# blyssprivacy/sdk

Measured on NVIDIA H100. Metric: PIR server queries/sec (Spiral process_query), higher is better.
Workload: dtype u64

## Files before the change

### sdk_b200/build.py

```python
import os
import subprocess
import sys

HERE = os.path.dirname(os.path.abspath(__file__))
CSRC = os.path.join(HERE, "csrc")
SO = os.path.join(HERE, "libb200pir.so")
SOURCES = ["api.cu", "poly_kernels.cu", "mul_kernels.cu", "imma_kernels.cu", "wire_kernels.cu", "tc5_kernels.cu", "dpir_gemm.cu"]
HEADERS = ["common.cuh", "kernels.h", "ntt_core.cuh", "tc5_layout.cuh", "tc5_ptx.cuh", "ntt_core4096.cuh", "ntt_tables.hpp",
           "item_place.cuh", "update_body.hpp", os.path.join("..", "..", "include", "b200pir.h")]
NVCC_FLAGS = ["-gencode", "arch=compute_90a,code=sm_90a", "-lineinfo", "-O3", "-std=c++17", "--extended-lambda",
              "-Xcompiler", "-fPIC", "-ccbin", "/usr/bin/g++" if os.path.exists("/usr/bin/g++") else "g++"]


def _stale():
    if not os.path.exists(SO):
        return True
    t = os.path.getmtime(SO)
    return any(os.path.getmtime(os.path.join(CSRC, f)) > t for f in SOURCES + HEADERS)


def build(force=False, verbose=False):
    if not force and not _stale():
        return SO
    nvcc = os.environ.get("NVCC", "/usr/local/cuda/bin/nvcc")
    objs = []
    procs = []
    for src in SOURCES:
        obj = os.path.join(CSRC, src.replace(".cu", ".o"))
        cmd = [nvcc] + NVCC_FLAGS + (["-Xptxas", "-v"] if verbose else []) + ["-c", os.path.join(CSRC, src), "-o", obj]
        procs.append((src, subprocess.Popen(cmd, stdout=subprocess.PIPE, stderr=subprocess.STDOUT, text=True)))
        objs.append(obj)
    for src, p in procs:
        out, _ = p.communicate()
        if verbose or p.returncode:
            sys.stderr.write(out)
        if p.returncode:
            raise RuntimeError("nvcc failed on " + src)
    subprocess.check_call([nvcc, "-shared", "-gencode", "arch=compute_90a,code=sm_90a", "-o", SO] + objs + ["-ccbin", NVCC_FLAGS[-1]])
    return SO


if __name__ == "__main__":
    print(build(force="--force" in sys.argv, verbose="-v" in sys.argv))
```

### sdk_b200/csrc/poly_kernels.cu

```cuda
#include "kernels.h"
#include "ntt_core4096.cuh"

namespace b200pir {

namespace {

constexpr int CTA = 512;
constexpr int HI_TW = NTT_N - 64;

__constant__ Twiddle c_tw_lo[2][3][64];

struct TwConst {
  int n, dir;
  __device__ __forceinline__ Twiddle operator()(int i) const { return c_tw_lo[n][dir][i]; }
  __device__ __forceinline__ void load2(int i, Twiddle (&t)[2]) const { t[0] = (*this)(i); t[1] = (*this)(i + 1); }
  __device__ __forceinline__ void load4(int i, Twiddle (&t)[4]) const {
    t[0] = (*this)(i); t[1] = (*this)(i + 1); t[2] = (*this)(i + 2); t[3] = (*this)(i + 3);
  }
};
struct TwShared {
  const Twiddle* p;
  __device__ __forceinline__ Twiddle operator()(int i) const { return p[i - 64]; }
  __device__ __forceinline__ void load2(int i, Twiddle (&t)[2]) const {
    uint4 v = *reinterpret_cast<const uint4*>(p + (i - 64));
    t[0] = Twiddle{v.x, v.y}; t[1] = Twiddle{v.z, v.w};
  }
  __device__ __forceinline__ void load4(int i, Twiddle (&t)[4]) const {
    uint4 v = *reinterpret_cast<const uint4*>(p + (i - 64)), w = *(reinterpret_cast<const uint4*>(p + (i - 64)) + 1);
    t[0] = Twiddle{v.x, v.y}; t[1] = Twiddle{v.z, v.w}; t[2] = Twiddle{w.x, w.y}; t[3] = Twiddle{w.z, w.w};
  }
};
struct TwGlobal {
  const Twiddle* p;
  __device__ __forceinline__ Twiddle operator()(int i) const {
    uint2 v = __ldg(reinterpret_cast<const uint2*>(p + i));
    return Twiddle{v.x, v.y};
  }
  __device__ __forceinline__ void load2(int i, Twiddle (&t)[2]) const {
    uint4 v = __ldg(reinterpret_cast<const uint4*>(p + i));
    t[0] = Twiddle{v.x, v.y}; t[1] = Twiddle{v.z, v.w};
  }
  __device__ __forceinline__ void load4(int i, Twiddle (&t)[4]) const {
    uint4 v = __ldg(reinterpret_cast<const uint4*>(p + i)), w = __ldg(reinterpret_cast<const uint4*>(p + i) + 1);
    t[0] = Twiddle{v.x, v.y}; t[1] = Twiddle{v.z, v.w}; t[2] = Twiddle{w.x, w.y}; t[3] = Twiddle{w.z, w.w};
  }
};

struct Grp {
  int tid;
  int n;
  uint32_t q;
  uint64_t cr1;
  const Twiddle* fwd;
  const Twiddle* inv;
  const Twiddle* inv_lz;
  uint32_t* smem;
  uint32_t* smem2;
  const Twiddle* fwd_hi_sm;
};
struct CtaSync {
  __device__ __forceinline__ void operator()() const { __syncthreads(); }
};

__device__ __forceinline__ Grp make_grp(const DevParams& P, uint32_t* ntt_smem) {
  Grp g;
  g.n = threadIdx.x >> 8;
  g.tid = threadIdx.x & 255;
  g.q = g.n ? P.q[1] : P.q[0];
  g.cr1 = g.n ? P.cr1[1] : P.cr1[0];
  g.fwd = g.n ? P.fwd[1] : P.fwd[0];
  g.inv = g.n ? P.inv[1] : P.inv[0];
  g.inv_lz = g.n ? P.inv_lz[1] : P.inv_lz[0];
  g.smem = ntt_smem + g.n * NTT_SMEM_WORDS;
  g.smem2 = nullptr;
  g.fwd_hi_sm = nullptr;
  return g;
}
__device__ __forceinline__ Grp make_grp_single(const DevParams& P, uint32_t* ntt_smem, int n) {
  Grp g;
  g.n = n;
  g.tid = threadIdx.x;
  g.q = n ? P.q[1] : P.q[0];
  g.cr1 = n ? P.cr1[1] : P.cr1[0];
  g.fwd = n ? P.fwd[1] : P.fwd[0];
  g.inv = n ? P.inv[1] : P.inv[0];
  g.inv_lz = n ? P.inv_lz[1] : P.inv_lz[0];
  g.smem = ntt_smem;
  g.smem2 = nullptr;
  g.fwd_hi_sm = nullptr;
  return g;
}
__device__ __forceinline__ void stage_fwd_twiddles(Grp& g, Twiddle* dst) {
  for (int i = g.tid; i < HI_TW; i += 256) {
    uint2 v = __ldg(reinterpret_cast<const uint2*>(g.fwd + 64 + i));
    dst[i] = Twiddle{v.x, v.y};
  }
  g.fwd_hi_sm = dst;
// ... 57 lines not shown
      for (int a = 0; a < 8; a++) {
        const uint64_t va = v(a);
        x0[a] = gadget_digit_fast<BYTE>(va, k, bits, mask);
        x1[a] = gadget_digit_fast<BYTE>(va, k + 1, bits, mask);
      }
      ntt_forward_group2_lz<NTT_OUT_LAZY16>(g.tid, x0, x1, g.smem, g.smem2, TwConst{g.n, 0}, TwShared{g.fwd_hi_sm}, g.q, CtaSync());
      if (cnt + 2 > 16) { acc_reduce<ROWS>(acc, g); cnt = 1; }
      cnt += 2;
      const uint32_t* c = c0 + (size_t)k * col_step;
#pragma unroll
      for (int r = 0; r < ROWS; r++) {
        uint32_t cv[8];
        ld8_ro(cv, c + (size_t)r * row_step);
#pragma unroll
        for (int e = 0; e < 8; e++) acc[r][e] += (uint64_t)x0[e] * cv[e];
      }
#pragma unroll
      for (int r = 0; r < ROWS; r++) {
        uint32_t cv[8];
        ld8_ro(cv, c + col_step + (size_t)r * row_step);
#pragma unroll
        for (int e = 0; e < 8; e++) acc[r][e] += (uint64_t)x1[e] * cv[e];
      }
    }
  }
#pragma unroll 1
  for (; k < ndig; k++) {
    uint32_t x[8];
#pragma unroll
    for (int a = 0; a < 8; a++) x[a] = gadget_digit_fast<BYTE>(v(a), k, bits, mask);
    if (SM) ntt_forward_group_lz<NTT_OUT_LAZY16>(g.tid, x, g.smem, TwConst{g.n, 0}, TwShared{g.fwd_hi_sm}, g.q, CtaSync());
    else ntt_forward_group_lz<NTT_OUT_LAZY16>(g.tid, x, g.smem, TwConst{g.n, 0}, TwGlobal{g.fwd}, g.q, CtaSync());
    if (cnt + 1 > 16) { acc_reduce<ROWS>(acc, g); cnt = 1; }
    cnt += 1;
    const uint32_t* c = c0 + (size_t)k * col_step;
#pragma unroll
    for (int r = 0; r < ROWS; r++) {
      uint32_t cv[8];
      ld8_ro(cv, c + (size_t)r * row_step);
#pragma unroll
      for (int e = 0; e < 8; e++) acc[r][e] += (uint64_t)x[e] * cv[e];
    }
  }
}

template <int ROWS, bool SM, typename Coef>
__device__ __forceinline__ void digits_mac(uint64_t (&acc)[ROWS][8], int& cnt, Coef v, int ndig,
                                           int bits, const uint32_t* c0, size_t col_step, size_t row_step,
                                           const Grp& g) {
  if (bits == 8) digits_mac_impl<ROWS, SM, true>(acc, cnt, v, ndig, bits, c0, col_step, row_step, g);
  else digits_mac_impl<ROWS, SM, false>(acc, cnt, v, ndig, bits, c0, col_step, row_step, g);
}

template <typename Sink>
__device__ __forceinline__ void crt_lift(const uint32_t (&x)[8], uint32_t* res, const Grp& g, const DevParams& P,
                                         Sink sink) {
  __syncthreads();
#pragma unroll
  for (int a = 0; a < 8; a++) res[g.n * POLY + a * 256 + g.tid] = x[a];
  __syncthreads();
#pragma unroll
  for (int a4 = 0; a4 < 4; a4++) {
    int z = (g.n * 4 + a4) * 256 + g.tid;
    sink(z, crt_compose(res[z], res[POLY + z], P));
  }
}

__global__ void __launch_bounds__(256) k_ntt32(DevParams P, uint32_t* polys, int inverse) {
  __shared__ __align__(16) uint32_t ntt_smem[NTT_SMEM_WORDS];
  Grp g = make_grp_single(P, ntt_smem, blockIdx.y);
  uint32_t* p = polys + ((size_t)blockIdx.x * 2 + g.n) * POLY;
  uint32_t x[8];
  if (!inverse) {
#pragma unroll
    for (int a = 0; a < 8; a++) x[a] = p[a * 256 + g.tid];
    grp_ntt_fwd<false>(g, x);
    st8(p + g.tid * 8, x);
  } else {
    ld8(x, p + g.tid * 8);
    grp_ntt_inv(g, x);
#pragma unroll
    for (int a = 0; a < 8; a++) p[a * 256 + g.tid] = x[a];
  }
}
__global__ void __launch_bounds__(NTT4K_THREADS)
k_ntt32_4k(uint32_t q0, uint32_t q1, const Twiddle* __restrict__ tw , uint32_t* polys, int inverse) {
  __shared__ __align__(16) uint32_t sm[NTT4K_SMEM_WORDS];
  const int n = blockIdx.y, tid = threadIdx.x;
  const uint32_t q = n ? q1 : q0;
  uint32_t* p = polys + ((size_t)blockIdx.x * 2 + n) * NTT4K_N;
  const TwGlobal tab{tw + (size_t)(2 * n + (inverse ? 1 : 0)) * NTT4K_N};
  uint32_t x[8];
  if (!inverse) {
#pragma unroll
    for (int a = 0; a < 8; a++) x[a] = p[a * NTT4K_THREADS + tid];
    ntt4k_forward_group(tid, x, sm, tab, q, CtaSync());
    st8(p + tid * 8, x);
  } else {
    ld8(x, p + tid * 8);
    ntt4k_inverse_group(tid, x, sm, tab, q, CtaSync());
#pragma unroll
    for (int a = 0; a < 8; a++) p[a * NTT4K_THREADS + tid] = x[a];
  }
}
__global__ void __launch_bounds__(256) k_ntt_u64(DevParams P, uint64_t* polys, int inverse) {
  __shared__ __align__(16) uint32_t ntt_smem[NTT_SMEM_WORDS];
// ... 67 lines not shown
             size_t c_batch_stride, int slices_per_query, int t_gsw, int bits) {
  __shared__ __align__(16) uint32_t ntt_smem[2 * NTT_SMEM_WORDS];
  __shared__ uint32_t res[2 * POLY];
  Grp g = make_grp(P, ntt_smem);
  const int b = blockIdx.x / half, i = blockIdx.x % half;
  uint64_t* base = cts + (size_t)b * batch_stride;
  const size_t qoff = (size_t)(b / slices_per_query) * c_batch_stride;
  const int cols = 2 * t_gsw;
  const size_t col_step = (size_t)2 * 2 * POLY;
  const size_t row_step = (size_t)cols * 2 * POLY;

  uint64_t acc[2][8];
#pragma unroll
  for (int r = 0; r < 2; r++)
#pragma unroll
    for (int e = 0; e < 8; e++) acc[r][e] = 0;
  int cnt = 0;
#pragma unroll 1
  for (int src = 0; src < 2; src++) {
    const uint64_t* ct = base + (size_t)(src == 0 ? i : half + i) * 2 * POLY;
    const uint32_t* C = (src == 0 ? c_neg : c_pos) + qoff;
#pragma unroll 1
    for (int rho = 0; rho < 2; rho++) {
      uint64_t v[8];
#pragma unroll
      for (int a = 0; a < 8; a++) v[a] = ct[rho * POLY + a * 256 + g.tid];
      const uint32_t* c0 = C + ((size_t)rho * 2 + g.n) * POLY + g.tid * 8;
      digits_mac<2, false>(acc, cnt, RegCoef{v}, t_gsw, bits, c0, col_step, row_step, g);
    }
  }
  uint64_t* dst = base + (size_t)i * 2 * POLY;
#pragma unroll 1
  for (int r = 0; r < 2; r++) {
    uint32_t x[8];
#pragma unroll
    for (int e = 0; e < 8; e++) x[e] = barrett64(acc[r][e], g.cr1, g.q);
    grp_ntt_inv(g, x);
    uint64_t* d = dst + r * POLY;
    crt_lift(x, res, g, P, [&](int z, uint64_t val) { d[z] = val; });
  }
}

__device__ __forceinline__ uint32_t digit_diff(uint64_t vh, uint64_t vi, int k, int bits, uint64_t mask, uint32_t q) {
  return gadget_digit(vh, k, bits, mask) - gadget_digit(vi, k, bits, mask) + q;
}
__device__ __forceinline__ uint32_t byte_pair_diff(uint64_t vh, uint64_t vi, int k) {
  const uint32_t sel = 0x7070u | ((uint32_t)(k + 1) << 8) | (uint32_t)k;
  return __byte_perm((uint32_t)vh, (uint32_t)(vh >> 32), sel) + 0x01000100u -
         __byte_perm((uint32_t)vi, (uint32_t)(vi >> 32), sel);
}
constexpr int kFoldPlanes = 4;

template <bool BYTE>
__global__ void __launch_bounds__(256, 2)
k_fold_res_lz(DevParams P, const uint32_t* __restrict__ in, uint32_t* __restrict__ out, size_t batch_stride, int half,
              const uint32_t* __restrict__ c_pos, size_t c_batch_stride, int slices_per_query, int t_gsw, int bits,
              const uint32_t* __restrict__ zero_flags ) {
  if (zero_flags) {
    const int bz = blockIdx.x / half, iz = blockIdx.x % half;
    const uint32_t fa = zero_flags[(size_t)bz * 2 * half + iz], fb = zero_flags[(size_t)bz * 2 * half + half + iz];
    if (fa | fb) {
      const uint32_t* src = in + (size_t)bz * batch_stride + (size_t)((fa ? half : 0) + iz) * 4 * POLY;
      uint32_t* dst = out + (size_t)bz * batch_stride + (size_t)iz * 4 * POLY;
#pragma unroll
      for (int rho = 0; rho < 2; rho++) {
        uint32_t x[8];
        ld8_ro(x, src + ((size_t)rho * 2 + blockIdx.y) * POLY + threadIdx.x * 8);
        st8(dst + ((size_t)rho * 2 + blockIdx.y) * POLY + threadIdx.x * 8, x);
      }
      return;
    }
  }
  extern __shared__ __align__(16) uint8_t dyn_smem[];
  uint32_t* sm0 = reinterpret_cast<uint32_t*>(dyn_smem);
  uint32_t* sm1 = sm0 + NTT_SMEM_WORDS;
  Twiddle* tw = reinterpret_cast<Twiddle*>(sm1 + NTT_SMEM_WORDS);
  Grp g = make_grp_single(P, sm0, blockIdx.y);
  stage_fwd_twiddles(g, tw);
  const TwConst lo{g.n, 0};
  const TwShared hi{tw};
  const int b = blockIdx.x / half, i = blockIdx.x % half;
  const uint32_t* ci = in + (size_t)b * batch_stride + (size_t)i * 4 * POLY;
  const uint32_t* ch = in + (size_t)b * batch_stride + (size_t)(half + i) * 4 * POLY;
  const uint32_t* C = c_pos + (size_t)(b / slices_per_query) * c_batch_stride;
  const int cols = 2 * t_gsw;
  const size_t row_step = (size_t)cols * 2 * POLY;
  const uint64_t mask = (1ull << bits) - 1;
  const uint32_t q = g.q;
  uint32_t* planes = reinterpret_cast<uint32_t*>(tw + HI_TW) + g.tid;

  uint64_t acc[2][8];
#pragma unroll
  for (int r = 0; r < 2; r++)
#pragma unroll
    for (int e = 0; e < 8; e++) acc[r][e] = 0;
  int cnt = 0;
#pragma unroll 1
  for (int rho = 0; rho < 2; rho++) {
    uint64_t vi[8], vh[8];
#pragma unroll
    for (int a = 0; a < 8; a++) {
      const int z = a * 256 + g.tid;
      vi[a] = crt_compose(__ldg(ci + (rho * 2 + 0) * POLY + z), __ldg(ci + (rho * 2 + 1) * POLY + z), P);
      vh[a] = crt_compose(__ldg(ch + (rho * 2 + 0) * POLY + z), __ldg(ch + (rho * 2 + 1) * POLY + z), P);
      if (BYTE) {
#pragma unroll
        for (int p = 0; p < kFoldPlanes; p++)
          if (2 * p < t_gsw) planes[p * POLY + a * 256] = byte_pair_diff(vh[a], vi[a], 2 * p);
      }
    }
    const uint32_t* c0 = C + ((size_t)rho * 2 + g.n) * POLY + g.tid * 8;
    int k = 0;
#pragma unroll 1
    for (; k + 1 < t_gsw; k += 2) {
      uint32_t x0[8], x1[8];
#pragma unroll
      for (int a = 0; a < 8; a++) {
        if (BYTE) {
          const uint32_t w = planes[(k >> 1) * POLY + a * 256];
          x0[a] = (w & 0xffffu) + (q - 256u);
          x1[a] = (w >> 16) + (q - 256u);
        } else {
          x0[a] = digit_diff(vh[a], vi[a], k, bits, mask, q);
          x1[a] = digit_diff(vh[a], vi[a], k + 1, bits, mask, q);
        }
      }
      ntt_forward_group2_lz<NTT_OUT_LAZY16>(g.tid, x0, x1, sm0, sm1, lo, hi, q, CtaSync());
      if (cnt + 2 > 16) { acc_reduce<2>(acc, g); cnt = 1; }
      cnt += 2;
#pragma unroll
      for (int r = 0; r < 2; r++) {
        uint32_t cv[8];
        ld8_ro(cv, c0 + (size_t)r * row_step + (size_t)k * 4 * POLY);
#pragma unroll
        for (int e = 0; e < 8; e++) acc[r][e] += (uint64_t)x0[e] * cv[e];
      }
#pragma unroll
      for (int r = 0; r < 2; r++) {
        uint32_t cv[8];
        ld8_ro(cv, c0 + (size_t)r * row_step + (size_t)(k + 1) * 4 * POLY);
#pragma unroll
        for (int e = 0; e < 8; e++) acc[r][e] += (uint64_t)x1[e] * cv[e];
      }
    }
    if (k < t_gsw) {
      uint32_t x0[8];
#pragma unroll
      for (int a = 0; a < 8; a++)
        x0[a] = BYTE ? (planes[(k >> 1) * POLY + a * 256] & 0xffffu) + (q - 256u) : digit_diff(vh[a], vi[a], k, bits, mask, q);
      ntt_forward_group_lz<NTT_OUT_LAZY16>(g.tid, x0, sm0, lo, hi, q, CtaSync());
      if (cnt + 1 > 16) { acc_reduce<2>(acc, g); cnt = 1; }
      cnt += 1;
#pragma unroll
      for (int r = 0; r < 2; r++) {
        uint32_t cv[8];
        ld8_ro(cv, c0 + (size_t)r * row_step + (size_t)k * 4 * POLY);
#pragma unroll
        for (int e = 0; e < 8; e++) acc[r][e] += (uint64_t)x0[e] * cv[e];
      }
    }
  }
  uint32_t y0[8], y1[8];
#pragma unroll
  for (int e = 0; e < 8; e++) {
    y0[e] = barrett64(acc[0][e], g.cr1, q);
    y1[e] = barrett64(acc[1][e], g.cr1, q);
  }
  ntt_inverse_group2_nh(g.tid, y0, y1, sm0, sm1, TwConst{g.n, 2}, TwGlobal{g.inv_lz}, q, CtaSync());
  uint32_t* co = out + (size_t)b * batch_stride + (size_t)i * 4 * POLY;
#pragma unroll
  for (int a = 0; a < 8; a++) {
    const int z = a * 256 + g.tid;
    co[(0 * 2 + g.n) * POLY + z] = addmod(y0[a], __ldg(ci + (0 * 2 + g.n) * POLY + z), q);
    co[(1 * 2 + g.n) * POLY + z] = addmod(y1[a], __ldg(ci + (1 * 2 + g.n) * POLY + z), q);
  }
}

__global__ void __launch_bounds__(256)
k_ct_zero_flags(const uint32_t* __restrict__ cts, size_t batch_stride, int per_batch, uint32_t* __restrict__ flags) {
  const int b = blockIdx.x / per_batch, idx = blockIdx.x % per_batch;
  const uint4* p = reinterpret_cast<const uint4*>(cts + (size_t)b * batch_stride + (size_t)idx * 4 * POLY);
  uint32_t acc = 0;
#pragma unroll
  for (int k = 0; k < 8; k++) {
    const uint4 v = __ldg(p + k * 256 + threadIdx.x);
    acc |= v.x | v.y | v.z | v.w;
  }
  const int any = __syncthreads_or(acc != 0);
  if (threadIdx.x == 0) flags[blockIdx.x] = any ? 0u : 1u;
}

__global__ void k_folding_neg(DevParams P, uint32_t* out, const uint32_t* vf, size_t total, int t_gsw, int bits) {
  size_t idx = (size_t)blockIdx.x * blockDim.x + threadIdx.x;
  if (idx >= total) return;
  int n = (int)((idx / POLY) & 1);
  size_t poly = idx / (2 * POLY);
  int cols = 2 * t_gsw;
  int c = (int)(poly % cols);
  int r = (int)((poly / cols) & 1);
  uint32_t q = P.q[n];
  uint32_t v = vf[idx];
  uint32_t neg = v == 0 ? 0u : q - v;
  uint32_t gval = 0;
  if ((c & 1) == r) {
    int j = c >> 1;
    if (bits * j < 64) gval = barrett64(1ull << (bits * j), P.cr1[n], q);
  }
  out[idx] = addmod(neg, gval, q);
}

__global__ void k_expand_scalar(DevParams P, uint32_t* v, size_t v_stride, int num_in, const uint32_t* neg1) {
  v += (size_t)blockIdx.y * v_stride;
  size_t idx = (size_t)blockIdx.x * blockDim.x + threadIdx.x;
  size_t total = (size_t)num_in * 4 * POLY;
  if (idx >= total) return;
  int z = (int)(idx % POLY);
  int n = (int)((idx / POLY) & 1);
  uint32_t a = v[idx], b = neg1[n * POLY + z];
  v[total + idx] = barrett64((uint64_t)a * b, P.cr1[n], P.q[n]);
}

__global__ void __launch_bounds__(CTA, 1) k_expand_round(DevParams P, uint32_t* v, size_t v_stride, ExpandRound R) {
  v += (size_t)blockIdx.y * v_stride;
  extern __shared__ __align__(16) uint8_t dyn_smem[];
  uint32_t* ntt_smem = reinterpret_cast<uint32_t*>(dyn_smem);
  uint32_t* res = ntt_smem + 4 * NTT_SMEM_WORDS;
  uint64_t* autom = reinterpret_cast<uint64_t*>(res + 2 * POLY);
// ... 467 lines not shown

__device__ __forceinline__ uint64_t rescale_dev(uint64_t a, uint64_t inp_mod, uint64_t out_mod) {
  typedef __int128 i128;
  long long inp_mod_i = (long long)inp_mod;
  long long inp_val = (long long)(a % inp_mod);
  if (inp_val >= inp_mod_i / 2) inp_val -= inp_mod_i;
  long long sign = inp_val >= 0 ? 1 : -1;
  i128 val = (i128)inp_val * (i128)out_mod;
  i128 result = (val + (i128)(sign * (inp_mod_i / 2))) / (i128)inp_mod;
  i128 om = (i128)out_mod;
  result = (result + (i128)((inp_mod / out_mod) * out_mod) + 2 * om) % om;
  return (uint64_t)((result + om) % om);
}
__global__ void k_encode(DevParams P, uint64_t* out, size_t out_words, const uint64_t* packed, size_t packed_q_stride, int n,
                         int instances, uint64_t q2, int q2_bits, uint64_t q1, int q1_bits) {
  size_t w = (size_t)blockIdx.x * blockDim.x + threadIdx.x;
  if (w >= out_words) return;
  out += (size_t)blockIdx.y * out_words;
  packed += (size_t)blockIdx.y * packed_q_stride;
  const uint64_t first_cnt = (uint64_t)n * POLY, rest_cnt = (uint64_t)n * n * POLY;
  const uint64_t inst_bits = first_cnt * q2_bits + rest_cnt * q1_bits;
  uint64_t lo_bit = (uint64_t)w * 64, hi_bit = lo_bit + 64;
  uint64_t word = 0;
  uint64_t bit = lo_bit;
  while (bit < hi_bit) {
    uint64_t inst = bit / inst_bits;
    if (inst >= (uint64_t)instances) break;
    uint64_t off = bit - inst * inst_bits;
    const uint64_t* pk = packed + inst * (uint64_t)(n + 1) * n * POLY;
    uint64_t vstart, val;
    int vb;
    if (off < first_cnt * q2_bits) {
      uint64_t vi = off / q2_bits;
      vstart = inst * inst_bits + vi * q2_bits;
      vb = q2_bits;
      val = rescale_dev(pk[vi], P.modulus, q2);
    } else {
      uint64_t o2 = off - first_cnt * q2_bits;
      uint64_t vi = o2 / q1_bits;
      vstart = inst * inst_bits + first_cnt * q2_bits + vi * q1_bits;
      vb = q1_bits;
      val = rescale_dev(pk[first_cnt + vi], P.modulus, q1);
    }
    val &= (vb >= 64) ? ~0ull : ((1ull << vb) - 1);
    if (vstart >= lo_bit) word |= val << (vstart - lo_bit);
    else word |= val >> (lo_bit - vstart);
    bit = vstart + vb;
  }
  out[w] = word;
}

inline unsigned grid1d(size_t total, int block) { return (unsigned)((total + block - 1) / block); }
const size_t kDynSmemBig = (size_t)(4 * NTT_SMEM_WORDS + 2 * POLY) * 4 + (size_t)2 * POLY * 8 + (size_t)2 * HI_TW * 8;
const size_t kDynSmemFold = (size_t)(2 * NTT_SMEM_WORDS) * 4 + (size_t)HI_TW * 8;

}

void upload_poly_constants(const Twiddle* lo ) {
  B200_CUDA(cudaMemcpyToSymbol(c_tw_lo, lo, sizeof(Twiddle) * 2 * 3 * 64));
}
void launch_ntt_u64(const DevParams& P, uint64_t* polys, size_t count, bool inverse, cudaStream_t s) {
  if (count) ++g_kernel_launches, k_ntt_u64<<<dim3((unsigned)count, 2), 256, 0, s>>>(P, polys, inverse ? 1 : 0);
}
void launch_ntt32(const DevParams& P, uint32_t* polys, size_t count, bool inverse, cudaStream_t s) {
  if (count) ++g_kernel_launches, k_ntt32<<<dim3((unsigned)count, 2), 256, 0, s>>>(P, polys, inverse ? 1 : 0);
}
void launch_ntt32_4k(uint32_t q0, uint32_t q1, const Twiddle* tw, uint32_t* polys, size_t count, bool inverse, cudaStream_t s) {
  if (count) ++g_kernel_launches, k_ntt32_4k<<<dim3((unsigned)count, 2), NTT4K_THREADS, 0, s>>>(q0, q1, tw, polys, inverse ? 1 : 0);
}
void launch_to_ntt(const DevParams& P, uint32_t* out, const uint64_t* raw, size_t count, cudaStream_t s) {
  if (count) ++g_kernel_launches, k_to_ntt<<<dim3((unsigned)count, 2), 256, 0, s>>>(P, out, raw, 0, 0);
}
void launch_to_ntt_strided(const DevParams& P, uint32_t* out, size_t out_stride, const uint64_t* raw, size_t raw_stride,
                           size_t count, int batches, cudaStream_t s) {
  if (count && batches)
    ++g_kernel_launches, k_to_ntt<<<dim3((unsigned)count, 2, (unsigned)batches), 256, 0, s>>>(P, out, raw, out_stride, raw_stride);
}
void launch_raw_to_res(const DevParams& P, uint32_t* out, const uint64_t* raw, size_t polys, cudaStream_t s) {
  if (polys) ++g_kernel_launches, k_raw_to_res<<<grid1d(polys * POLY, 256), 256, 0, s>>>(P, out, raw, polys);
}
void launch_res_to_raw(const DevParams& P, uint64_t* out, const uint32_t* res, size_t polys, cudaStream_t s) {
  if (polys) ++g_kernel_launches, k_res_to_raw<<<grid1d(polys * POLY, 256), 256, 0, s>>>(P, out, res, polys);
}
void launch_fold_res(const DevParams& P, const uint32_t* in, uint32_t* out, size_t batch, size_t batch_stride, int half,
                     const uint32_t* c_pos, size_t c_batch_stride, int slices_per_query, int t_gsw, int bits,
                     uint32_t* zero_flags, cudaStream_t s) {
  if (batch == 0 || half == 0) return;
  if (zero_flags) {
    ++g_kernel_launches;
    k_ct_zero_flags<<<(unsigned)(batch * 2 * half), 256, 0, s>>>(in, batch_stride, 2 * half, zero_flags);
  }
  ++g_kernel_launches;
  const dim3 grid((unsigned)(batch * half), 2);
  const bool byte = bits == 8 && t_gsw <= 2 * kFoldPlanes;
  const size_t smem = kDynSmemFold + (byte ? (size_t)kFoldPlanes * POLY * 4 : 0);
  auto kern = byte ? k_fold_res_lz<true> : k_fold_res_lz<false>;
  opt_in_smem(kern, (int)smem);
  kern<<<grid, 256, smem, s>>>(P, in, out, batch_stride, half, c_pos, c_batch_stride, slices_per_query, t_gsw, bits, zero_flags);
}
void launch_from_ntt(const DevParams& P, uint64_t* out_raw, const uint32_t* in, size_t count, cudaStream_t s) {
  if (count) ++g_kernel_launches, k_from_ntt<<<(unsigned)count, CTA, 0, s>>>(P, out_raw, in);
}
void launch_widen(uint64_t* out, const uint32_t* in, size_t words, cudaStream_t s) {
  if (words) ++g_kernel_launches, k_widen<<<grid1d(words, 256), 256, 0, s>>>(out, in, words);
}
void launch_narrow(uint32_t* out, const uint64_t* in, size_t words, cudaStream_t s) {
  if (words) ++g_kernel_launches, k_narrow<<<grid1d(words, 256), 256, 0, s>>>(out, in, words);
}
void launch_fold_round(const DevParams& P, uint64_t* cts, size_t batch, size_t batch_stride, int half,
                       const uint32_t* c_pos, const uint32_t* c_neg, size_t c_batch_stride, int slices_per_query,
                       int t_gsw, int bits, cudaStream_t s) {
  if (batch == 0 || half == 0) return;
  ++g_kernel_launches;
  k_fold_round<<<(unsigned)(batch * half), CTA, 0, s>>>(P, cts, batch_stride, half, c_pos, c_neg, c_batch_stride,
                                                        slices_per_query, t_gsw, bits);
}
void launch_folding_neg(const DevParams& P, uint32_t* out, const uint32_t* v_folding, int count, int t_gsw, int bits,
                        cudaStream_t s) {
  size_t total = (size_t)count * 2 * 2 * t_gsw * 2 * POLY;
  if (total) ++g_kernel_launches, k_folding_neg<<<grid1d(total, 256), 256, 0, s>>>(P, out, v_folding, total, t_gsw, bits);
}
void launch_expand_scalar(const DevParams& P, uint32_t* v, size_t v_stride, int nq, int num_in, const uint32_t* neg1_r,
                          cudaStream_t s) {
  size_t total = (size_t)num_in * 4 * POLY;
  ++g_kernel_launches;
  k_expand_scalar<<<dim3(grid1d(total, 256), nq), 256, 0, s>>>(P, v, v_stride, num_in, neg1_r);
}
void launch_expand_round(const DevParams& P, uint32_t* v, size_t v_stride, int nq, const ExpandRound& R, cudaStream_t s) {
  opt_in_smem(k_expand_round, (int)kDynSmemBig);
  ++g_kernel_launches;
  k_expand_round<<<dim3((unsigned)(2 * R.num_in), nq), CTA, kDynSmemBig, s>>>(P, v, v_stride, R);
}
void launch_expand_round_pair(const DevParams& P, uint32_t* v, size_t v_stride, int nq, const ExpandRound& R,
                              const uint32_t* neg1_r, cudaStream_t s) {
  opt_in_smem(k_expand_round_pair, (int)kDynSmemBig);
  ++g_kernel_launches;
  k_expand_round_pair<<<dim3((unsigned)R.num_in, nq), CTA, kDynSmemBig, s>>>(P, v, v_stride, R, neg1_r);
}
void launch_expand_round_res(const DevParams& P, uint32_t* v, size_t v_stride, uint32_t* xr, size_t xr_stride, int nq,
                             const ExpandRound& R, const uint32_t* neg1_r, cudaStream_t s) {
  const size_t smem = (size_t)2 * NTT_SMEM_WORDS * 4 + (size_t)POLY * 8 + (size_t)HI_TW * 8;
  opt_in_smem(k_expand_round_res, (int)smem);
  g_kernel_launches += 2;
  k_expand_intt<<<dim3((unsigned)R.num_in, 2, nq), 256, 0, s>>>(P, v, v_stride, xr, xr_stride, R);
  k_expand_round_res<<<dim3((unsigned)R.num_in, 2, nq), 256, smem, s>>>(P, v, v_stride, xr, xr_stride, R, neg1_r);
}
void launch_reorient(const MulGeom& G, uint4* q_dev, size_t q_stride, const uint32_t* v, size_t v_stride, int nq,
                     int idx_factor, cudaStream_t s) {
  size_t total = (size_t)G.dim0 * POLY;
  ++g_kernel_launches;
  k_reorient<<<dim3(grid1d(total, 256), nq), 256, 0, s>>>(G, q_dev, q_stride, v, v_stride, idx_factor);
// ... 41 lines not shown
```

Baseline: 1495.

## Rewrite fold kernel with 128-thread radix-16 NTT holding 16 coefficients per thread

Adds a new three-pass radix-16 NTT core in which 128 threads each hold 16 coefficients, and ports the fold kernel onto it. The kernel previously used 256 threads with 8 coefficients each. Only the last-stage twiddles are staged in shared memory, and the non-byte path parks the composed 64-bit values in shared memory instead of registers. The aim is fewer shared-memory passes and barriers per NTT and more work per thread. The costs are higher register pressure with 16-wide accumulators, fewer threads per block, and the inverse NTTs running one row at a time instead of paired.

```diff
diff --git a/sdk_b200/build.py b/sdk_b200/build.py
--- a/sdk_b200/build.py
+++ b/sdk_b200/build.py
@@ -6,7 +6,7 @@
 CSRC = os.path.join(HERE, "csrc")
 SO = os.path.join(HERE, "libb200pir.so")
 SOURCES = ["api.cu", "poly_kernels.cu", "mul_kernels.cu", "imma_kernels.cu", "wire_kernels.cu", "tc5_kernels.cu", "dpir_gemm.cu"]
-HEADERS = ["common.cuh", "kernels.h", "ntt_core.cuh", "tc5_layout.cuh", "tc5_ptx.cuh", "ntt_core4096.cuh", "ntt_tables.hpp",
+HEADERS = ["common.cuh", "kernels.h", "ntt_core.cuh", "ntt_core16.cuh", "tc5_layout.cuh", "tc5_ptx.cuh", "ntt_core4096.cuh", "ntt_tables.hpp",
            "item_place.cuh", "update_body.hpp", os.path.join("..", "..", "include", "b200pir.h")]
 NVCC_FLAGS = ["-gencode", "arch=compute_90a,code=sm_90a", "-lineinfo", "-O3", "-std=c++17", "--extended-lambda",
               "-Xcompiler", "-fPIC", "-ccbin", "/usr/bin/g++" if os.path.exists("/usr/bin/g++") else "g++"]
diff --git a/sdk_b200/csrc/ntt_core16.cuh b/sdk_b200/csrc/ntt_core16.cuh
--- /dev/null
+++ b/sdk_b200/csrc/ntt_core16.cuh
@@ -0,0 +1,256 @@
+#pragma once
+#include "ntt_core.cuh"
+
+namespace b200pir {
+
+static const int NTT16_THREADS = 128;
+static const int NTT16_SMEM_WORDS = 2048 + 4 * 64 + 8 * 16;
+static const int NTT16_C_CHUNKS = 7;
+
+NTT_HD int ntt16_phys(int e) { return e + 4 * (e >> 5) + 8 * (e >> 7); }
+NTT_HD int ntt16_c_entry(int c, int tid) {
+  return c == 0 ? 256 + 2 * tid : (c < 3 ? 512 + 4 * tid + 2 * (c - 1) : 1024 + 8 * tid + 2 * (c - 3));
+}
+
+struct Ntt16Addr {
+  int a, b, c;
+};
+NTT_HD Ntt16Addr ntt16_addr(int tid) {
+  return Ntt16Addr{tid + 4 * (tid >> 5), 152 * (tid >> 3) + (tid & 7), 16 * tid + 4 * (tid >> 1) + 8 * (tid >> 3)};
+}
+NTT_HD int ntt16_off_b(int j) { return 8 * j + 4 * (j >> 2); }
+
+struct TwChunksArray {
+  const Twiddle* p;
+  int tid;
+  NTT_HD void operator()(int c, Twiddle (&t)[2]) const {
+    const int i = ntt16_c_entry(c, tid);
+    t[0] = p[i];
+    t[1] = p[i + 1];
+  }
+};
+
+template <bool MID, typename Tab>
+NTT_HD void radix16_fwd_lz(uint32_t (&x)[16], Tab tab, int m0, int g0, uint32_t q, uint32_t two_q) {
+  {
+    const Twiddle t0 = tab(m0 + g0);
+#pragma unroll
+    for (int j = 0; j < 8; j++) bfly_fwd_lz(x[j], x[j + 8], t0, q, two_q);
+  }
+  {
+    Twiddle t1[2];
+    tab.load2(2 * m0 + 2 * g0, t1);
+#pragma unroll
+    for (int h = 0; h < 2; h++)
+#pragma unroll
+      for (int j = 0; j < 4; j++) bfly_fwd_lz(x[8 * h + j], x[8 * h + j + 4], t1[h], q, two_q);
+  }
+  {
+    Twiddle t2[4];
+    tab.load4(4 * m0 + 4 * g0, t2);
+#pragma unroll
+    for (int h = 0; h < 4; h++)
+#pragma unroll
+      for (int j = 0; j < 2; j++) bfly_fwd_lz(x[4 * h + j], x[4 * h + j + 2], t2[h], q, two_q);
+  }
+  if (MID) {
+#pragma unroll
+    for (int j = 0; j < 16; j++) x[j] = ntt_c8(x[j], 4 * two_q);
+  }
+  {
+#pragma unroll
+    for (int u = 0; u < 2; u++) {
+      Twiddle t3[4];
+      tab.load4(8 * m0 + 8 * g0 + 4 * u, t3);
+#pragma unroll
+      for (int h = 0; h < 4; h++) bfly_fwd_lz(x[8 * u + 2 * h], x[8 * u + 2 * h + 1], t3[h], q, two_q);
+    }
+  }
+}
+
+template <bool IN4Q, typename Tab>
+NTT_HD void fwd16_pass_a(const Ntt16Addr& ad, uint32_t (&x)[16], uint32_t* smem, Tab tab, uint32_t q, uint32_t two_q) {
+  if (IN4Q) {
+#pragma unroll
+    for (int j = 0; j < 16; j++) x[j] = ntt_min(x[j], x[j] - two_q);
+  }
+  radix16_fwd_lz<false>(x, tab, 1, 0, q, two_q);
+#pragma unroll
+  for (int j = 0; j < 16; j++) smem[ad.a + 152 * j] = x[j];
+}
+template <typename Tab>
+NTT_HD void fwd16_pass_b(int tid, const Ntt16Addr& ad, uint32_t (&x)[16], uint32_t* smem, Tab tab, uint32_t q, uint32_t two_q) {
+#pragma unroll
+  for (int j = 0; j < 16; j++) x[j] = smem[ad.b + ntt16_off_b(j)];
+  radix16_fwd_lz<true>(x, tab, 16, tid >> 3, q, two_q);
+#pragma unroll
+  for (int j = 0; j < 16; j++) smem[ad.b + ntt16_off_b(j)] = x[j];
+}
+template <int OUT, typename Chunks>
+NTT_HD void fwd16_pass_c(const Ntt16Addr& ad, uint32_t (&x)[16], const uint32_t* smem, Chunks ch, uint32_t q, uint32_t two_q) {
+#pragma unroll
+  for (int k = 0; k < 16; k++) x[k] = smem[ad.c + k];
+  {
+    Twiddle t8[2];
+    ch(0, t8);
+#pragma unroll
+    for (int h = 0; h < 2; h++)
+#pragma unroll
+      for (int k = 0; k < 4; k++) bfly_fwd_lz(x[8 * h + k], x[8 * h + k + 4], t8[h], q, two_q);
+  }
+#pragma unroll
+  for (int h = 0; h < 2; h++) {
+    Twiddle t9[2];
+    ch(1 + h, t9);
+#pragma unroll
+    for (int g = 0; g < 2; g++)
+#pragma unroll
+      for (int k = 0; k < 2; k++) bfly_fwd_lz(x[8 * h + 4 * g + k], x[8 * h + 4 * g + k + 2], t9[g], q, two_q);
+  }
+#pragma unroll
+  for (int c = 0; c < 4; c++) {
+    Twiddle t10[2];
+    ch(3 + c, t10);
+#pragma unroll
+    for (int g = 0; g < 2; g++) bfly_fwd_lz(x[4 * c + 2 * g], x[4 * c + 2 * g + 1], t10[g], q, two_q);
+  }
+  if (OUT >= NTT_OUT_LAZY4) {
+#pragma unroll
+    for (int k = 0; k < 16; k++) { x[k] = ntt_min(x[k], x[k] - 4 * two_q); x[k] = ntt_min(x[k], x[k] - 2 * two_q); }
+  }
+  if (OUT == NTT_OUT_CANON) {
+#pragma unroll
+    for (int k = 0; k < 16; k++) x[k] = ntt_canon(x[k], q, two_q);
+  }
+}
+
+template <typename Chunks>
+NTT_HD void inv16_pass_c(const Ntt16Addr& ad, uint32_t (&x)[16], uint32_t* smem, Chunks ch, uint32_t q, uint32_t two_q) {
+  const uint32_t eight_q = 4 * two_q;
+#pragma unroll
+  for (int c = 0; c < 4; c++) {
+    Twiddle t10[2];
+    ch(3 + c, t10);
+#pragma unroll
+    for (int g = 0; g < 2; g++) bfly_inv_nh<false>(x[4 * c + 2 * g], x[4 * c + 2 * g + 1], t10[g], q, two_q, 0);
+  }
+#pragma unroll
+  for (int h = 0; h < 2; h++) {
+    Twiddle t9[2];
+    ch(1 + h, t9);
+#pragma unroll
+    for (int g = 0; g < 2; g++)
+#pragma unroll
+      for (int k = 0; k < 2; k++)
+        bfly_inv_nh<false>(x[8 * h + 4 * g + k], x[8 * h + 4 * g + k + 2], t9[g], q, 2 * two_q, 0);
+  }
+  {
+    Twiddle t8[2];
+    ch(0, t8);
+#pragma unroll
+    for (int h = 0; h < 2; h++)
+#pragma unroll
+      for (int k = 0; k < 4; k++) bfly_inv_nh<true>(x[8 * h + k], x[8 * h + k + 4], t8[h], q, eight_q, eight_q);
+  }
+#pragma unroll
+  for (int k = 0; k < 16; k++) smem[ad.c + k] = x[k];
+}
+template <typename Tab>
+NTT_HD void radix16_inv_nh(uint32_t (&x)[16], Tab tab, int m0, int g0, uint32_t q, uint32_t eight_q) {
+  {
+#pragma unroll
+    for (int u = 0; u < 2; u++) {
+      Twiddle t3[4];
+      tab.load4(8 * m0 + 8 * g0 + 4 * u, t3);
+#pragma unroll
+      for (int h = 0; h < 4; h++) bfly_inv_nh<true>(x[8 * u + 2 * h], x[8 * u + 2 * h + 1], t3[h], q, eight_q, eight_q);
+    }
+  }
+  {
+    Twiddle t2[4];
+    tab.load4(4 * m0 + 4 * g0, t2);
+#pragma unroll
+    for (int h = 0; h < 4; h++)
+#pragma unroll
+      for (int j = 0; j < 2; j++) bfly_inv_nh<true>(x[4 * h + j], x[4 * h + j + 2], t2[h], q, eight_q, eight_q);
+  }
+  {
+    Twiddle t1[2];
+    tab.load2(2 * m0 + 2 * g0, t1);
+#pragma unroll
+    for (int h = 0; h < 2; h++)
+#pragma unroll
+      for (int j = 0; j < 4; j++) bfly_inv_nh<true>(x[8 * h + j], x[8 * h + j + 4], t1[h], q, eight_q, eight_q);
+  }
+  if (m0 > 1) {
+    const Twiddle t0 = tab(m0 + g0);
+#pragma unroll
+    for (int j = 0; j < 8; j++) bfly_inv_nh<true>(x[j], x[j + 8], t0, q, eight_q, eight_q);
+  }
+}
+template <typename Tab>
+NTT_HD void inv16_pass_b(int tid, const Ntt16Addr& ad, uint32_t (&x)[16], uint32_t* smem, Tab tab, uint32_t q, uint32_t two_q) {
+#pragma unroll
+  for (int j = 0; j < 16; j++) x[j] = smem[ad.b + ntt16_off_b(j)];
+  radix16_inv_nh(x, tab, 16, tid >> 3, q, 4 * two_q);
+#pragma unroll
+  for (int j = 0; j < 16; j++) smem[ad.b + ntt16_off_b(j)] = x[j];
+}
+template <typename Tab>
+NTT_HD void inv16_pass_a(const Ntt16Addr& ad, uint32_t (&x)[16], const uint32_t* smem, Tab tab, uint32_t q, uint32_t two_q) {
+#pragma unroll
+  for (int j = 0; j < 16; j++) x[j] = smem[ad.a + 152 * j];
+  const uint32_t eight_q = 4 * two_q;
+  radix16_inv_nh(x, tab, 1, 0, q, eight_q);
+  const Twiddle ninv = tab(0), w1s = tab(1);
+#pragma unroll
+  for (int j = 0; j < 8; j++) {
+    NTT_RC_SUM(x[j], x[j + 8]);
+    const uint32_t s = x[j] + x[j + 8], tt = x[j] - x[j + 8] + eight_q;
+    const uint32_t u = ntt_shoup(s, ninv, q), v = ntt_shoup(tt, w1s, q);
+    x[j] = ntt_min(u, u - q);
+    x[j + 8] = ntt_min(v, v - q);
+  }
+}
+
+#if defined(__CUDACC__)
+template <int OUT, bool IN4Q = false, typename Sync, typename TabLo, typename TabMid, typename Chunks>
+__device__ __forceinline__ void ntt16_forward_lz(int tid, const Ntt16Addr& ad, uint32_t (&x)[16], uint32_t* smem, TabLo lo,
+                                                 TabMid mid, Chunks ch, uint32_t q, Sync gsync) {
+  const uint32_t two_q = 2 * q;
+  gsync();
+  fwd16_pass_a<IN4Q>(ad, x, smem, lo, q, two_q);
+  gsync();
+  fwd16_pass_b(tid, ad, x, smem, mid, q, two_q);
+  gsync();
+  fwd16_pass_c<OUT>(ad, x, smem, ch, q, two_q);
+}
+template <int OUT, bool IN4Q = false, typename Sync, typename TabLo, typename TabMid, typename Chunks>
+__device__ __forceinline__ void ntt16_forward2_lz(int tid, const Ntt16Addr& ad, uint32_t (&x0)[16], uint32_t (&x1)[16],
+                                                  uint32_t* smem0, uint32_t* smem1, TabLo lo, TabMid mid, Chunks ch,
+                                                  uint32_t q, Sync gsync) {
+  const uint32_t two_q = 2 * q;
+  gsync();
+  fwd16_pass_a<IN4Q>(ad, x0, smem0, lo, q, two_q);
+  fwd16_pass_a<IN4Q>(ad, x1, smem1, lo, q, two_q);
+  gsync();
+  fwd16_pass_b(tid, ad, x0, smem0, mid, q, two_q);
+  fwd16_pass_b(tid, ad, x1, smem1, mid, q, two_q);
+  gsync();
+  fwd16_pass_c<OUT>(ad, x0, smem0, ch, q, two_q);
+  fwd16_pass_c<OUT>(ad, x1, smem1, ch, q, two_q);
+}
+template <typename Sync, typename TabLo, typename TabMid, typename Chunks>
+__device__ __forceinline__ void ntt16_inverse_nh(int tid, const Ntt16Addr& ad, uint32_t (&x)[16], uint32_t* smem, TabLo lo,
+                                                 TabMid mid, Chunks ch, uint32_t q, Sync gsync) {
+  const uint32_t two_q = 2 * q;
+  gsync();
+  inv16_pass_c(ad, x, smem, ch, q, two_q);
+  gsync();
+  inv16_pass_b(tid, ad, x, smem, mid, q, two_q);
+  gsync();
+  inv16_pass_a(ad, x, smem, lo, q, two_q);
+}
+#endif
+
+}
diff --git a/sdk_b200/csrc/poly_kernels.cu b/sdk_b200/csrc/poly_kernels.cu
--- a/sdk_b200/csrc/poly_kernels.cu
+++ b/sdk_b200/csrc/poly_kernels.cu
@@ -1,5 +1,6 @@
 #include "kernels.h"
 #include "ntt_core4096.cuh"
+#include "ntt_core16.cuh"
 
 namespace b200pir {
 
@@ -43,6 +44,37 @@
   __device__ __forceinline__ void load4(int i, Twiddle (&t)[4]) const {
     uint4 v = __ldg(reinterpret_cast<const uint4*>(p + i)), w = __ldg(reinterpret_cast<const uint4*>(p + i) + 1);
     t[0] = Twiddle{v.x, v.y}; t[1] = Twiddle{v.z, v.w}; t[2] = Twiddle{w.x, w.y}; t[3] = Twiddle{w.z, w.w};
+  }
+};
+
+struct TwL1 {
+  const Twiddle* p;
+  __device__ __forceinline__ Twiddle operator()(int i) const {
+    const uint2 v = *reinterpret_cast<const uint2*>(p + i);
+    return Twiddle{v.x, v.y};
+  }
+  __device__ __forceinline__ void load2(int i, Twiddle (&t)[2]) const {
+    const uint4 v = *reinterpret_cast<const uint4*>(p + i);
+    t[0] = Twiddle{v.x, v.y}; t[1] = Twiddle{v.z, v.w};
+  }
+  __device__ __forceinline__ void load4(int i, Twiddle (&t)[4]) const {
+    const uint4 v = *reinterpret_cast<const uint4*>(p + i), w = *(reinterpret_cast<const uint4*>(p + i) + 1);
+    t[0] = Twiddle{v.x, v.y}; t[1] = Twiddle{v.z, v.w}; t[2] = Twiddle{w.x, w.y}; t[3] = Twiddle{w.z, w.w};
+  }
+};
+struct TwChunksShared {
+  const uint4* p;
+  __device__ __forceinline__ void operator()(int c, Twiddle (&t)[2]) const {
+    const uint4 v = p[c * NTT16_THREADS];
+    t[0] = Twiddle{v.x, v.y}; t[1] = Twiddle{v.z, v.w};
+  }
+};
+struct TwChunksGlobal {
+  const Twiddle* p;
+  int tid;
+  __device__ __forceinline__ void operator()(int c, Twiddle (&t)[2]) const {
+    const uint4 v = __ldg(reinterpret_cast<const uint4*>(p + ntt16_c_entry(c, tid)));
+    t[0] = Twiddle{v.x, v.y}; t[1] = Twiddle{v.z, v.w};
   }
 };
 
@@ -206,6 +238,83 @@
   else digits_mac_impl<ROWS, SM, false>(acc, cnt, v, ndig, bits, c0, col_step, row_step, g);
 }
 
+struct Grp16 {
+  int tid, n;
+  uint32_t q;
+  uint64_t cr1;
+  const Twiddle* fwd;
+  const Twiddle* inv_lz;
+  Ntt16Addr ad;
+  uint32_t* smem;
+  uint32_t* smem2;
+  const uint4* tw_c;
+};
+constexpr size_t kSmemTwC16 = (size_t)NTT16_C_CHUNKS * NTT16_THREADS * 16;
+constexpr size_t kSmemNtt16 = (size_t)2 * NTT16_SMEM_WORDS * 4 + kSmemTwC16;
+
+__device__ __forceinline__ Grp16 make_grp16(const DevParams& P, uint32_t* smem) {
+  Grp16 g;
+  g.n = blockIdx.y;
+  g.tid = threadIdx.x;
+  g.q = g.n ? P.q[1] : P.q[0];
+  g.cr1 = g.n ? P.cr1[1] : P.cr1[0];
+  g.fwd = g.n ? P.fwd[1] : P.fwd[0];
+  g.inv_lz = g.n ? P.inv_lz[1] : P.inv_lz[0];
+  g.ad = ntt16_addr(g.tid);
+  g.smem = smem;
+  g.smem2 = nullptr;
+  g.tw_c = nullptr;
+  return g;
+}
+__device__ __forceinline__ void stage_c_twiddles16(Grp16& g, uint4* dst) {
+#pragma unroll
+  for (int c = 0; c < NTT16_C_CHUNKS; c++)
+    dst[c * NTT16_THREADS + g.tid] = __ldg(reinterpret_cast<const uint4*>(g.fwd + ntt16_c_entry(c, g.tid)));
+  g.tw_c = dst + g.tid;
+}
+template <int OUT>
+__device__ __forceinline__ void grp16_fwd(const Grp16& g, uint32_t (&x)[16]) {
+  ntt16_forward_lz<OUT>(g.tid, g.ad, x, g.smem, TwConst{g.n, 0}, TwL1{g.fwd}, TwChunksShared{g.tw_c}, g.q, CtaSync());
+}
+template <int OUT>
+__device__ __forceinline__ void grp16_fwd2(const Grp16& g, uint32_t (&x0)[16], uint32_t (&x1)[16]) {
+  ntt16_forward2_lz<OUT>(g.tid, g.ad, x0, x1, g.smem, g.smem2, TwConst{g.n, 0}, TwL1{g.fwd}, TwChunksShared{g.tw_c}, g.q,
+                         CtaSync());
+}
+__device__ __forceinline__ void grp16_inv(const Grp16& g, uint32_t (&x)[16]) {
+  ntt16_inverse_nh(g.tid, g.ad, x, g.smem, TwConst{g.n, 2}, TwGlobal{g.inv_lz}, TwChunksGlobal{g.inv_lz, g.tid}, g.q, CtaSync());
+}
+__device__ __forceinline__ void ld16_ro(uint32_t (&x)[16], const uint32_t* p) {
+#pragma unroll
+  for (int c = 0; c < 4; c++) {
+    const uint4 v = __ldg(reinterpret_cast<const uint4*>(p) + c);
+    x[4 * c] = v.x; x[4 * c + 1] = v.y; x[4 * c + 2] = v.z; x[4 * c + 3] = v.w;
+  }
+}
+__device__ __forceinline__ void st16(uint32_t* p, const uint32_t (&x)[16]) {
+#pragma unroll
+  for (int c = 0; c < 4; c++) reinterpret_cast<uint4*>(p)[c] = make_uint4(x[4 * c], x[4 * c + 1], x[4 * c + 2], x[4 * c + 3]);
+}
+template <int ROWS>
+__device__ __forceinline__ void acc_reduce16(uint64_t (&acc)[ROWS][16], uint64_t cr1, uint32_t q) {
+#pragma unroll
+  for (int r = 0; r < ROWS; r++)
+#pragma unroll
+    for (int k = 0; k < 16; k++) acc[r][k] = barrett64(acc[r][k], cr1, q);
+}
+template <int ROWS>
+__device__ __forceinline__ void mac16(uint64_t (&acc)[ROWS][16], const uint32_t (&x)[16], const uint32_t* c, size_t row_step) {
+#pragma unroll
+  for (int r = 0; r < ROWS; r++)
+#pragma unroll
+    for (int c4 = 0; c4 < 4; c4++) {
+      const uint4 v = __ldg(reinterpret_cast<const uint4*>(c + (size_t)r * row_step) + c4);
+      acc[r][4 * c4 + 0] += (uint64_t)x[4 * c4 + 0] * v.x;
+      acc[r][4 * c4 + 1] += (uint64_t)x[4 * c4 + 1] * v.y;
+      acc[r][4 * c4 + 2] += (uint64_t)x[4 * c4 + 2] * v.z;
+      acc[r][4 * c4 + 3] += (uint64_t)x[4 * c4 + 3] * v.w;
+    }
+}
 template <typename Sink>
 __device__ __forceinline__ void crt_lift(const uint32_t (&x)[8], uint32_t* res, const Grp& g, const DevParams& P,
                                          Sink sink) {
@@ -379,7 +488,7 @@
 constexpr int kFoldPlanes = 4;
 
 template <bool BYTE>
-__global__ void __launch_bounds__(256, 2)
+__global__ void __launch_bounds__(NTT16_THREADS, 3)
 k_fold_res_lz(DevParams P, const uint32_t* __restrict__ in, uint32_t* __restrict__ out, size_t batch_stride, int half,
               const uint32_t* __restrict__ c_pos, size_t c_batch_stride, int slices_per_query, int t_gsw, int bits,
               const uint32_t* __restrict__ zero_flags ) {
@@ -391,115 +500,95 @@
       uint32_t* dst = out + (size_t)bz * batch_stride + (size_t)iz * 4 * POLY;
 #pragma unroll
       for (int rho = 0; rho < 2; rho++) {
-        uint32_t x[8];
-        ld8_ro(x, src + ((size_t)rho * 2 + blockIdx.y) * POLY + threadIdx.x * 8);
-        st8(dst + ((size_t)rho * 2 + blockIdx.y) * POLY + threadIdx.x * 8, x);
+        uint32_t x[16];
+        ld16_ro(x, src + ((size_t)rho * 2 + blockIdx.y) * POLY + threadIdx.x * 16);
+        st16(dst + ((size_t)rho * 2 + blockIdx.y) * POLY + threadIdx.x * 16, x);
       }
       return;
     }
   }
   extern __shared__ __align__(16) uint8_t dyn_smem[];
-  uint32_t* sm0 = reinterpret_cast<uint32_t*>(dyn_smem);
-  uint32_t* sm1 = sm0 + NTT_SMEM_WORDS;
-  Twiddle* tw = reinterpret_cast<Twiddle*>(sm1 + NTT_SMEM_WORDS);
-  Grp g = make_grp_single(P, sm0, blockIdx.y);
-  stage_fwd_twiddles(g, tw);
-  const TwConst lo{g.n, 0};
-  const TwShared hi{tw};
+  uint32_t* xs = reinterpret_cast<uint32_t*>(dyn_smem);
+  uint4* twc = reinterpret_cast<uint4*>(xs + 2 * NTT16_SMEM_WORDS);
+  Grp16 g = make_grp16(P, xs);
+  g.smem2 = xs + NTT16_SMEM_WORDS;
+  stage_c_twiddles16(g, twc);
   const int b = blockIdx.x / half, i = blockIdx.x % half;
-  const uint32_t* ci = in + (size_t)b * batch_stride + (size_t)i * 4 * POLY;
-  const uint32_t* ch = in + (size_t)b * batch_stride + (size_t)(half + i) * 4 * POLY;
+  const size_t ct_off = (size_t)b * batch_stride + (size_t)i * 4 * POLY;
+  const uint32_t* ci = in + ct_off;
+  const uint32_t* ch = ci + (size_t)half * 4 * POLY;
   const uint32_t* C = c_pos + (size_t)(b / slices_per_query) * c_batch_stride;
-  const int cols = 2 * t_gsw;
-  const size_t row_step = (size_t)cols * 2 * POLY;
+  const int row_step = 2 * t_gsw * 2 * POLY;
   const uint64_t mask = (1ull << bits) - 1;
   const uint32_t q = g.q;
-  uint32_t* planes = reinterpret_cast<uint32_t*>(tw + HI_TW) + g.tid;
-
-  uint64_t acc[2][8];
+  uint32_t* planes = reinterpret_cast<uint32_t*>(twc + NTT16_C_CHUNKS * NTT16_THREADS) + g.tid;
+  uint64_t* parked = reinterpret_cast<uint64_t*>(twc + NTT16_C_CHUNKS * NTT16_THREADS) + g.tid;
+
+  uint64_t acc[2][16];
 #pragma unroll
   for (int r = 0; r < 2; r++)
 #pragma unroll
-    for (int e = 0; e < 8; e++) acc[r][e] = 0;
+    for (int e = 0; e < 16; e++) acc[r][e] = 0;
   int cnt = 0;
 #pragma unroll 1
   for (int rho = 0; rho < 2; rho++) {
-    uint64_t vi[8], vh[8];
-#pragma unroll
-    for (int a = 0; a < 8; a++) {
-      const int z = a * 256 + g.tid;
-      vi[a] = crt_compose(__ldg(ci + (rho * 2 + 0) * POLY + z), __ldg(ci + (rho * 2 + 1) * POLY + z), P);
-      vh[a] = crt_compose(__ldg(ch + (rho * 2 + 0) * POLY + z), __ldg(ch + (rho * 2 + 1) * POLY + z), P);
+#pragma unroll 4
+    for (int j = 0; j < 16; j++) {
+      const int z = j * NTT16_THREADS + g.tid;
+      const uint64_t vi = crt_compose(__ldg(ci + (rho * 2 + 0) * POLY + z), __ldg(ci + (rho * 2 + 1) * POLY + z), P);
+      const uint64_t vh = crt_compose(__ldg(ch + (rho * 2 + 0) * POLY + z), __ldg(ch + (rho * 2 + 1) * POLY + z), P);
       if (BYTE) {
 #pragma unroll
         for (int p = 0; p < kFoldPlanes; p++)
-          if (2 * p < t_gsw) planes[p * POLY + a * 256] = byte_pair_diff(vh[a], vi[a], 2 * p);
+          if (2 * p < t_gsw) planes[p * POLY + j * NTT16_THREADS] = byte_pair_diff(vh, vi, 2 * p);
+      } else {
+        parked[j * NTT16_THREADS] = vi;
+        parked[POLY + j * NTT16_THREADS] = vh;
       }
     }
-    const uint32_t* c0 = C + ((size_t)rho * 2 + g.n) * POLY + g.tid * 8;
+    const int c0 = (rho * 2 + g.n) * POLY + g.tid * 16;
     int k = 0;
 #pragma unroll 1
-    for (; k + 1 < t_gsw; k += 2) {
-      uint32_t x0[8], x1[8];
-#pragma unroll
-      for (int a = 0; a < 8; a++) {
-        if (BYTE) {
-          const uint32_t w = planes[(k >> 1) * POLY + a * 256];
-          x0[a] = (w & 0xffffu) + (q - 256u);
-          x1[a] = (w >> 16) + (q - 256u);
-        } else {
-          x0[a] = digit_diff(vh[a], vi[a], k, bits, mask, q);
-          x1[a] = digit_diff(vh[a], vi[a], k + 1, bits, mask, q);
-        }
+    for (; BYTE && k + 1 < t_gsw; k += 2) {
+      uint32_t x0[16], x1[16];
+#pragma unroll
+      for (int j = 0; j < 16; j++) {
+        const uint32_t w = planes[(k >> 1) * POLY + j * NTT16_THREADS];
+        x0[j] = (w & 0xffffu) + (q - 256u);
+        x1[j] = (w >> 16) + (q - 256u);
       }
-      ntt_forward_group2_lz<NTT_OUT_LAZY16>(g.tid, x0, x1, sm0, sm1, lo, hi, q, CtaSync());
-      if (cnt + 2 > 16) { acc_reduce<2>(acc, g); cnt = 1; }
+      grp16_fwd2<NTT_OUT_LAZY16>(g, x0, x1);
+      if (cnt + 2 > 16) { acc_reduce16<2>(acc, blockIdx.y ? P.cr1[1] : P.cr1[0], q); cnt = 1; }
       cnt += 2;
-#pragma unroll
-      for (int r = 0; r < 2; r++) {
-        uint32_t cv[8];
-        ld8_ro(cv, c0 + (size_t)r * row_step + (size_t)k * 4 * POLY);
-#pragma unroll
-        for (int e = 0; e < 8; e++) acc[r][e] += (uint64_t)x0[e] * cv[e];
-      }
-#pragma unroll
-      for (int r = 0; r < 2; r++) {
-        uint32_t cv[8];
-        ld8_ro(cv, c0 + (size_t)r * row_step + (size_t)(k + 1) * 4 * POLY);
-#pragma unroll
-        for (int e = 0; e < 8; e++) acc[r][e] += (uint64_t)x1[e] * cv[e];
-      }
-    }
-    if (k < t_gsw) {
-      uint32_t x0[8];
-#pragma unroll
-      for (int a = 0; a < 8; a++)
-        x0[a] = BYTE ? (planes[(k >> 1) * POLY + a * 256] & 0xffffu) + (q - 256u) : digit_diff(vh[a], vi[a], k, bits, mask, q);
-      ntt_forward_group_lz<NTT_OUT_LAZY16>(g.tid, x0, sm0, lo, hi, q, CtaSync());
-      if (cnt + 1 > 16) { acc_reduce<2>(acc, g); cnt = 1; }
+      mac16<2>(acc, x0, C + c0 + k * 4 * POLY, row_step);
+      mac16<2>(acc, x1, C + c0 + (k + 1) * 4 * POLY, row_step);
+    }
+#pragma unroll 1
+    for (; k < t_gsw; k++) {
+      uint32_t x[16];
+#pragma unroll
+      for (int j = 0; j < 16; j++)
+        x[j] = BYTE ? (planes[(k >> 1) * POLY + j * NTT16_THREADS] & 0xffffu) + (q - 256u)
+                    : digit_diff(parked[POLY + j * NTT16_THREADS], parked[j * NTT16_THREADS], k, bits, mask, q);
+      grp16_fwd<NTT_OUT_LAZY16>(g, x);
+      if (cnt + 1 > 16) { acc_reduce16<2>(acc, blockIdx.y ? P.cr1[1] : P.cr1[0], q); cnt = 1; }
       cnt += 1;
-#pragma unroll
-      for (int r = 0; r < 2; r++) {
-        uint32_t cv[8];
-        ld8_ro(cv, c0 + (size_t)r * row_step + (size_t)k * 4 * POLY);
-#pragma unroll
-        for (int e = 0; e < 8; e++) acc[r][e] += (uint64_t)x0[e] * cv[e];
-      }
-    }
-  }
-  uint32_t y0[8], y1[8];
-#pragma unroll
-  for (int e = 0; e < 8; e++) {
-    y0[e] = barrett64(acc[0][e], g.cr1, q);
-    y1[e] = barrett64(acc[1][e], g.cr1, q);
-  }
-  ntt_inverse_group2_nh(g.tid, y0, y1, sm0, sm1, TwConst{g.n, 2}, TwGlobal{g.inv_lz}, q, CtaSync());
-  uint32_t* co = out + (size_t)b * batch_stride + (size_t)i * 4 * POLY;
-#pragma unroll
-  for (int a = 0; a < 8; a++) {
-    const int z = a * 256 + g.tid;
-    co[(0 * 2 + g.n) * POLY + z] = addmod(y0[a], __ldg(ci + (0 * 2 + g.n) * POLY + z), q);
-    co[(1 * 2 + g.n) * POLY + z] = addmod(y1[a], __ldg(ci + (1 * 2 + g.n) * POLY + z), q);
+      mac16<2>(acc, x, C + c0 + k * 4 * POLY, row_step);
+      if (BYTE) break;
+    }
+  }
+  uint32_t* co = out + ct_off;
+#pragma unroll 1
+  for (int r = 0; r < 2; r++) {
+    uint32_t y[16];
+#pragma unroll
+    for (int e = 0; e < 16; e++) y[e] = barrett64(r ? acc[1][e] : acc[0][e], g.cr1, q);
+    grp16_inv(g, y);
+#pragma unroll
+    for (int j = 0; j < 16; j++) {
+      const int z = j * NTT16_THREADS + g.tid;
+      co[(r * 2 + g.n) * POLY + z] = addmod(y[j], __ldg(ci + (r * 2 + g.n) * POLY + z), q);
+    }
   }
 }
 
@@ -1073,7 +1162,7 @@
 
 inline unsigned grid1d(size_t total, int block) { return (unsigned)((total + block - 1) / block); }
 const size_t kDynSmemBig = (size_t)(4 * NTT_SMEM_WORDS + 2 * POLY) * 4 + (size_t)2 * POLY * 8 + (size_t)2 * HI_TW * 8;
-const size_t kDynSmemFold = (size_t)(2 * NTT_SMEM_WORDS) * 4 + (size_t)HI_TW * 8;
+const size_t kDynSmemFold = kSmemNtt16 + (size_t)kFoldPlanes * POLY * 4;
 
 }
 
@@ -1114,10 +1203,9 @@
   ++g_kernel_launches;
   const dim3 grid((unsigned)(batch * half), 2);
   const bool byte = bits == 8 && t_gsw <= 2 * kFoldPlanes;
-  const size_t smem = kDynSmemFold + (byte ? (size_t)kFoldPlanes * POLY * 4 : 0);
   auto kern = byte ? k_fold_res_lz<true> : k_fold_res_lz<false>;
-  opt_in_smem(kern, (int)smem);
-  kern<<<grid, 256, smem, s>>>(P, in, out, batch_stride, half, c_pos, c_batch_stride, slices_per_query, t_gsw, bits, zero_flags);
+  opt_in_smem(kern, (int)kDynSmemFold);
+  kern<<<grid, NTT16_THREADS, kDynSmemFold, s>>>(P, in, out, batch_stride, half, c_pos, c_batch_stride, slices_per_query, t_gsw, bits, zero_flags);
 }
 void launch_from_ntt(const DevParams& P, uint64_t* out_raw, const uint32_t* in, size_t count, cudaStream_t s) {
   if (count) ++g_kernel_launches, k_from_ntt<<<(unsigned)count, CTA, 0, s>>>(P, out_raw, in);
```

New measurement: 1522 (median of 6 runs). 1.9% higher.
